# halide/Halide

Measured on AMD Instinct MI355X. Metric: megapixels/sec local_laplacian 8-level fp32 4K, higher is better.
Workload: dtype f32; 1 GPU; apps/local_laplacian J=8 levels=8 alpha=1/7 beta=1, u16 RGB planar 3840x2160; distinct_frames_per_gpu=8, lut_cached=True, streams_per_gpu=4, frame_scheduling=4 frame-queue streams, boundary=C ABI local_laplacian(halide_buffer_t*,int32,float,float,halide_buffer_t*), rccl_ranks=1, parallelism=frames sharded over 1 GPU(s), no data-path collective

## Files before the change

### halide_amd/csrc/local_laplacian.hip

```cpp
#include "hlmi_device_math.h"
#include "hlmi_internal.h"

#include <atomic>
#include <mutex>
#include <optional>
#include <stdlib.h>
#include <string.h>
#include <type_traits>

using namespace hlmi;

namespace {

constexpr int J = 8;
constexpr int MAX_K = 32;
constexpr int STRIP = 126;
constexpr int KCH = 8;
constexpr int D0_THREADS = 256;

struct Level {
    int lox, loy;
    int w, h;
    int ws;
    size_t ps;
// ... 10 lines not shown
#define LL_PROBE_T(var) const unsigned long long var = wall_clock64()
#define LL_PROBE_ADD(slot, val) do { if ((threadIdx.x & 63) == 0) atomicAdd(&g_probe[slot], (unsigned long long)(val)); } while (0)
#else
#define LL_PROBE_T(var)
#define LL_PROBE_ADD(slot, val)
#endif

#ifndef HLMI_LL_RESIDENCY
#define HLMI_LL_RESIDENCY 0
#endif
#if HLMI_LL_RESIDENCY
__device__ int g_res[2][4096];
__device__ unsigned long long g_res_hist[16];
struct ResidencyProbe {
    int kind, slot;
    bool on;
    __device__ explicit ResidencyProbe(int k) : kind(k), slot(0), on(threadIdx.x == 0) {
        if (on) {
            unsigned hw, xcc;
            asm volatile("s_getreg_b32 %0, hwreg(HW_REG_HW_ID)" : "=s"(hw));
            asm volatile("s_getreg_b32 %0, hwreg(HW_REG_XCC_ID)" : "=s"(xcc));
            slot = (int)(((xcc & 0xfu) << 8) | ((hw >> 8) & 0xffu));
            const int own = atomicAdd(&g_res[kind][slot], 1);
            const int other = atomicAdd(&g_res[1 - kind][slot], 0);
            atomicAdd(&g_res_hist[8 * kind + min(other, 3)], 1ull);
            atomicAdd(&g_res_hist[8 * kind + 4 + min(own, 3)], 1ull);
        }
    }
    __device__ ~ResidencyProbe() {
        if (on) atomicSub(&g_res[kind][slot], 1);
    }
};
#define LL_RESIDENCY(kind) ResidencyProbe residency_probe_(kind)
#else
#define LL_RESIDENCY(kind)
#endif

struct Geometry {
    int K, half;
    float Km1, inv_Km1;
    int ix0, ix1, iy0, iy1;
};

__global__ void ll_remap_lut(float *lut, int half, float alpha) {
    int i = blockIdx.x * blockDim.x + threadIdx.x;
    if (i > 2 * half) return;
    float fx = (float)(i - half) * (1.0f / 256.0f);
    lut[i] = (alpha * fx) * dev::halide_exp(((-fx) * fx) * 0.5f);
}

__device__ __forceinline__ int xcd_block() {
    const int nb8 = gridDim.x >> 3, b = blockIdx.x;
    return (b < (nb8 << 3)) ? (b & 7) * nb8 + (b >> 3) : b;
}

__device__ __forceinline__ float down4(float a, float b, float c, float d) {
    return (dev::mad(3.0f, b + c, a) + d) * 0.125f;
}
__device__ __forceinline__ float down4_raw(float a, float b, float c, float d) { return dev::mad(3.0f, b + c, a) + d; }
__device__ __forceinline__ float down4_tail(float a, float b, float c, float d) {
    return (dev::mad(3.0f, b + c, a) + d) * 0.015625f;
}

__device__ __forceinline__ float gray_from(uint16_t r, uint16_t g, uint16_t b) {
    constexpr float s = (float)(1.0 / 65535.0);
    constexpr float C0 = (float)((double)s * (double)0.299f), C1 = (float)((double)s * (double)0.587f),
                    C2 = (float)((double)s * (double)0.114f);
    return dev::mad((float)b, C2, dev::mad2((float)r, C0, (float)g, C1));
// ... 1158 lines not shown
            nc = row(2 * T + 3);
            nd = row(2 * T + 4);
        }
        float dy[4] = {down4_raw(ra.x, rb.x, rc.x, rd.x), down4_raw(ra.y, rb.y, rc.y, rd.y), down4_raw(ra.z, rb.z, rc.z, rd.z),
                       down4_raw(ra.w, rb.w, rc.w, rd.w)};
        float2 o = hpair<ODD>(dy);
        if (store_ok) *reinterpret_cast<float2 *>(dp + (size_t)t * a.dws) = o;
        ra = rc, rb = rd, rc = nc, rd = nd;
    }
}
template<bool ODD>
__global__ __launch_bounds__(256) void ll_down_strip(StripArgs a) {
    const int wave = __builtin_amdgcn_readfirstlane(threadIdx.x >> 6);
    const int unit = xcd_block() * 4 + wave;
    if (unit >= a.nunits) return;
    down_strip_unit<ODD>(a, unit, threadIdx.x & 63);
}

constexpr int S2_RPU = 2;
constexpr int S2_NT = 2 * S2_RPU + 2;
constexpr int S2_NSRC = 2 * S2_NT + 2;
struct Strip2Args {
    const float *src;
    int slox, sloy, sw, sh, sws;
    size_t sps;
    float *g1;
    int so1, loy1, w1, h1, ws1;
    size_t ps1;
    float *g2;
    int so2, loy2, w2, h2, ws2;
    size_t ps2;
    int Pbase, S2, nsx, nsy, nunits;
};
template<bool ODD0, bool ODD1>
__global__ __launch_bounds__(256) void ll_down_strip2(Strip2Args p) {
    const int wave = __builtin_amdgcn_readfirstlane(threadIdx.x >> 6);
    const int unit = xcd_block() * 4 + wave;
    if (unit >= p.nunits) return;
    const int lane = threadIdx.x & 63;
    const int sy = unit % p.nsy, rest = unit / p.nsy, sx = rest % p.nsx, plane = rest / p.nsx;
    const int A = p.loy2 + sy * S2_RPU, B = min(A + S2_RPU - 1, p.loy2 + p.h2 - 1);
    const int P = p.Pbase + 2 * p.S2 * sx + 2 * lane;
    const QuadSel qs = quad_sel((ODD0 ? 2 * P - 1 : 2 * P - 2) - p.slox, p.sw);
    const bool edge_wave = __any(!qs.plain);
    const int T0 = 2 * A - 1;
    const int Ts0 = max(2 * A, p.loy1), Ts1 = min(2 * B + 1, p.loy1 + p.h1 - 1);
    const int off1 = P - p.so1;
    const bool st1_ok = lane < p.S2 && off1 >= 0 && off1 < p.w1;
    const int X2 = ODD1 ? (P + 1) >> 1 : P >> 1;
    const int off2 = X2 - p.so2;
    const bool st2_ok = (ODD1 ? lane < p.S2 : (lane >= 1 && lane <= p.S2)) && off2 >= 0 && off2 < p.w2;
    const float *sp = p.src + (size_t)plane * p.sps + qs.oq;
    float4 r[S2_NSRC];
#pragma unroll
    for (int i = 0; i < S2_NSRC; i++) r[i] = *reinterpret_cast<const float4 *>(sp + (size_t)dev::clampi(2 * T0 - 1 + i - p.sloy, 0, p.sh - 1) * p.sws);
    if (edge_wave) {
#pragma unroll
        for (int i = 0; i < S2_NSRC; i++) {
            const float4 v = r[i];
            r[i] = make_float4(pick4(v.x, v.y, v.z, v.w, qs.sel[0]), pick4(v.x, v.y, v.z, v.w, qs.sel[1]),
                               pick4(v.x, v.y, v.z, v.w, qs.sel[2]), pick4(v.x, v.y, v.z, v.w, qs.sel[3]));
        }
    }
    float *d1 = p.g1 + (size_t)plane * p.ps1 + off1, *d2 = p.g2 + (size_t)plane * p.ps2 + off2;
    float2 s0 = make_float2(0.0f, 0.0f), s1 = s0, pc = s0;
#pragma unroll
    for (int t = 0; t < S2_NT; t++) {
        const int T = T0 + t;
        const float4 a = r[2 * t], b = r[2 * t + 1], c = r[2 * t + 2], d = r[2 * t + 3];
        const float dy[4] = {down4_raw(a.x, b.x, c.x, d.x), down4_raw(a.y, b.y, c.y, d.y), down4_raw(a.z, b.z, c.z, d.z),
                             down4_raw(a.w, b.w, c.w, d.w)};
        const float2 res = hpair<ODD0>(dy);
        if (T >= Ts0 && T <= Ts1 && st1_ok) *reinterpret_cast<float2 *>(d1 + (size_t)(T - p.loy1) * p.ws1) = res;
        if ((t & 1) == 0) {
            pc.x = dev::mad(3.0f, s1.x + res.x, s0.x);
            pc.y = dev::mad(3.0f, s1.y + res.y, s0.y);
            s0 = res;
        } else {
            const float rx = pc.x + res.x, ry = pc.y + res.y;
            float o;
            if (ODD1) {
                const float nx = lane_next(rx), ny = lane_next(ry);
                o = down4_tail(rx, ry, nx, ny);
            } else {
                const float py = lane_prev(ry), nx = lane_next(rx);
                o = down4_tail(py, rx, ry, nx);
            }
            const int Y = (T - 2) >> 1;
            if (T >= 2 * A + 2 && Y <= B && st2_ok) d2[(size_t)(Y - p.loy2) * p.ws2] = o;
            s1 = res;
        }
    }
}


__device__ __forceinline__ float top_value(const float *__restrict__ g, size_t ps, size_t o, int K, float Km1) {
    float level = g[(size_t)K * ps + o] * Km1;
    int li = dev::clampi((int)level, 0, K - 2);
    float lf = level - (float)li;
    return dev::mad2(1.0f - lf, g[(size_t)li * ps + o], lf, g[(size_t)(li + 1) * ps + o]);
}
template<bool SEL = false>
__device__ __forceinline__ float outl_value(const float *__restrict__ g, int ws, size_t ps, int lox, int loy,
                                            const float *__restrict__ gc, int cws, size_t cps, int clox, int cloy,
                                            int X, int Y, int K, float Km1) {
    size_t o = (size_t)(Y - loy) * ws + (X - lox);
    float level = g[(size_t)K * ps + o] * Km1;
    int li = dev::clampi((int)level, 0, K - 2);
    float lf = level - (float)li;
    float l0 = g[(SEL ? 0 : (size_t)li * ps) + o] - up_at(gc + (size_t)li * cps, clox, cloy, cws, X, Y);
    float l1 = g[(SEL ? ps : (size_t)(li + 1) * ps) + o] - up_at(gc + (size_t)(li + 1) * cps, clox, cloy, cws, X, Y);
    return dev::mad2(1.0f - lf, l0, lf, l1);
}

__global__ void ll_top(const float *__restrict__ g, int ws, size_t ps, int lox, int loy, int rx0, int ry0, int rw,
                       int rh, int K, float Km1, float *__restrict__ out) {
    int x = blockIdx.x * blockDim.x + threadIdx.x, y = blockIdx.y;
    if (x >= rw || y >= rh) return;
    size_t o = (size_t)(ry0 + y - loy) * ws + (rx0 + x - lox);
    out[o] = top_value(g, ps, o, K, Km1);
}

// ... 17 lines not shown
    float outL = outl_value<SEL>(a.g, a.ws, a.ps, a.lox, a.loy, a.gc, a.cws, a.cps, a.clox, a.cloy, X, Y, a.K, a.Km1);
    a.out[o] = up_at(a.outc, a.clox, a.cloy, a.cws, X, Y) + outL;
}
template<bool SEL = false>
__global__ __launch_bounds__(256) void ll_up(UpArgs a) {
    up_pixel<SEL>(a, blockIdx.x * blockDim.x + threadIdx.x, blockIdx.y);
}
__global__ __launch_bounds__(256) void ll_up_outl(UpArgs a) {
    const int x = blockIdx.x * blockDim.x + threadIdx.x, y = blockIdx.y;
    if (x >= a.rw || y >= a.rh) return;
    const int X = a.rx0 + x, Y = a.ry0 + y;
    const size_t o = (size_t)(Y - a.loy) * a.ws + (X - a.lox);
    a.out[o] = up_at(a.outc, a.clox, a.cloy, a.cws, X, Y) + a.g[o];
}

struct DevLevel {
    float *g, *out;
    int lox, loy, w, h, ws;
    unsigned ps;
    int rx0, ry0, rw, rh;
};
struct CoarseArgs {
    DevLevel lv[J];
    int K;
    float Km1;
};

constexpr int DM_T = 4;
__host__ __device__ constexpr int dm_win(int depth_below) {
    int w = DM_T;
    for (int i = 0; i < depth_below; i++) w = 2 * w + 2;
    return w;
}
struct Range2 { int x0, x1, y0, y1; };
__device__ __forceinline__ Range2 clamp_to_box(const DevLevel &L, int x0, int x1, int y0, int y1) {
    Range2 r;
    r.x0 = dev::clampi(x0, L.lox, L.lox + L.w - 1), r.x1 = dev::clampi(x1, L.lox, L.lox + L.w - 1);
    r.y0 = dev::clampi(y0, L.loy, L.loy + L.h - 1), r.y1 = dev::clampi(y1, L.loy, L.loy + L.h - 1);
    return r;
}
template<int DEPTH>
__device__ __forceinline__ void down_multi_tile(const CoarseArgs &a, int ntx, int nty, int b) {
    constexpr int W1 = dm_win(DEPTH - 1), W2 = DEPTH >= 2 ? dm_win(DEPTH - 2) : 1, W3 = DEPTH >= 3 ? dm_win(DEPTH - 3) : 1,
                  W4 = DEPTH >= 4 ? dm_win(DEPTH - 4) : 1;
    __shared__ float tile1[W1 * W1], tile2[W2 * W2], tile3[W3 * W3], tile4[W4 * W4];
    float *const tiles[5] = {nullptr, tile1, tile2, tile3, tile4};
    const int ws_[5] = {0, W1, W2, W3, W4};
    const int tx = b % ntx, ty = (b / ntx) % nty, plane = b / (ntx * nty);
    Range2 win[5], own[5];
    {
        const DevLevel &T = a.lv[DEPTH];
        win[DEPTH] = own[DEPTH] = clamp_to_box(T, T.lox + tx * DM_T, T.lox + tx * DM_T + DM_T - 1, T.loy + ty * DM_T,
                                               T.loy + ty * DM_T + DM_T - 1);
#pragma unroll
        for (int d = DEPTH - 1; d >= 1; d--) {
            const DevLevel &L = a.lv[d];
            win[d] = clamp_to_box(L, 2 * win[d + 1].x0 - 1, 2 * win[d + 1].x1 + 2, 2 * win[d + 1].y0 - 1, 2 * win[d + 1].y1 + 2);
            own[d] = clamp_to_box(L, 2 * own[d + 1].x0, 2 * own[d + 1].x1 + 1, 2 * own[d + 1].y0, 2 * own[d + 1].y1 + 1);
        }
    }
#pragma unroll
    for (int d = 1; d <= DEPTH; d++) {
        const DevLevel &L = a.lv[d], &Sx = a.lv[d - 1];
        const Range2 w = win[d], o = own[d];
        const int nx = w.x1 - w.x0 + 1, n = nx * (w.y1 - w.y0 + 1);
        float *const dst = tiles[d];
        const float *const src_g = Sx.g + (size_t)plane * Sx.ps;
        const float *const src_t = tiles[d - 1];
        const Range2 pw = win[d == 1 ? 1 : d - 1];
        const int pnx = ws_[d == 1 ? 1 : d - 1];
        for (int e0 = threadIdx.x; e0 < n; e0 += 512) {
            float r[2][4][4];
            int X[2], Y[2], yy[2];
            bool ok[2];
#pragma unroll
            for (int u = 0; u < 2; u++) {
                const int e = e0 + 256 * u, ec = min(e, n - 1);
                ok[u] = e < n;
                yy[u] = ec / nx, X[u] = w.x0 + (ec - yy[u] * nx), Y[u] = w.y0 + yy[u];
#pragma unroll
                for (int i = 0; i < 4; i++) {
#pragma unroll
                    for (int k = 0; k < 4; k++) {
                        const int qx = dev::clampi(2 * X[u] - 1 + i, Sx.lox, Sx.lox + Sx.w - 1);
                        const int qy = dev::clampi(2 * Y[u] - 1 + k, Sx.loy, Sx.loy + Sx.h - 1);
                        r[u][i][k] = (d == 1) ? src_g[(size_t)(qy - Sx.loy) * Sx.ws + (qx - Sx.lox)]
                                              : src_t[(qy - pw.y0) * pnx + (qx - pw.x0)];
                    }
                }
            }
#pragma unroll
            for (int u = 0; u < 2; u++) {
                float v[4];
#pragma unroll
                for (int i = 0; i < 4; i++) v[i] = down4_raw(r[u][i][0], r[u][i][1], r[u][i][2], r[u][i][3]);
                const float val = down4_tail(v[0], v[1], v[2], v[3]);
                if (ok[u]) {
                    dst[yy[u] * ws_[d] + (X[u] - w.x0)] = val;
                    if (X[u] >= o.x0 && X[u] <= o.x1 && Y[u] >= o.y0 && Y[u] <= o.y1) {
                        L.g[(size_t)plane * L.ps + (size_t)(Y[u] - L.loy) * L.ws + (X[u] - L.lox)] = val;
                    }
                }
            }
        }
        if (d < DEPTH) __syncthreads();
    }
}
template<int DEPTH>
__global__ __launch_bounds__(256) void ll_down_multi(CoarseArgs a, int ntx, int nty) {
    down_multi_tile<DEPTH>(a, ntx, nty, (int)blockIdx.x);
}

constexpr int UM_T = 16;
__host__ __device__ constexpr int um_win(int d) {
    int w = UM_T;
    for (int i = 0; i < d; i++) w = w / 2 + 2;
    return w;
}
__host__ __device__ constexpr int um_off(int d) {
    int o = 0;
    for (int i = 0; i < d; i++) o += um_win(i) * um_win(i);
    return o;
}
static_assert(UM_T * UM_T <= 256 && um_win(1) * um_win(1) <= 256, "ll_up_multi: a level's region of a tile exceeds the workgroup");
template<int TOP>
__device__ __forceinline__ void up_multi_tile(const CoarseArgs &a, int ntx, int b) {
    __shared__ float tl[um_off(TOP + 1)];
    const int tx = b % ntx, ty = b / ntx;
    Range2 reg[TOP + 1];
    {
        const DevLevel &L = a.lv[0];
        reg[0].x0 = L.rx0 + tx * UM_T, reg[0].x1 = min(reg[0].x0 + UM_T - 1, L.rx0 + L.rw - 1);
        reg[0].y0 = L.ry0 + ty * UM_T, reg[0].y1 = min(reg[0].y0 + UM_T - 1, L.ry0 + L.rh - 1);
#pragma unroll
        for (int d = 1; d <= TOP; d++) {
            reg[d].x0 = dev::fdiv2(reg[d - 1].x0 - 1), reg[d].x1 = dev::fdiv2(reg[d - 1].x1 + 1);
            reg[d].y0 = dev::fdiv2(reg[d - 1].y0 - 1), reg[d].y1 = dev::fdiv2(reg[d - 1].y1 + 1);
        }
    }
    int eX[TOP + 1], eY[TOP + 1];
    bool act[TOP + 1];
    size_t eo[TOP + 1];
    float lvl[TOP + 1];
#pragma unroll
    for (int d = 0; d <= TOP; d++) {
        const DevLevel &L = a.lv[d];
        const Range2 r = reg[d];
        const int nx = r.x1 - r.x0 + 1, n = nx * (r.y1 - r.y0 + 1);
        act[d] = (int)threadIdx.x < n;
        const int e = act[d] ? (int)threadIdx.x : 0, yy = e / nx;
        eX[d] = r.x0 + (e - yy * nx), eY[d] = r.y0 + yy;
        eo[d] = (size_t)(eY[d] - L.loy) * L.ws + (eX[d] - L.lox);
        lvl[d] = L.g[(size_t)a.K * L.ps + eo[d]];
    }
    __builtin_amdgcn_sched_barrier(0);
    float lf[TOP + 1], g0[TOP + 1], g1[TOP + 1];
    int lis[TOP + 1];
    UpTaps t0[TOP + 1], t1[TOP + 1];
    auto planes_of = [&](int d) {
        const float level = lvl[d] * a.Km1;
        lis[d] = dev::clampi((int)level, 0, a.K - 2);
        lf[d] = level - (float)lis[d];
    };
#pragma unroll
    for (int d = 0; d <= TOP; d++) {
        const DevLevel &L = a.lv[d];
        planes_of(d);
        const int li = lis[d];
        g0[d] = L.g[(size_t)li * L.ps + eo[d]], g1[d] = L.g[(size_t)(li + 1) * L.ps + eo[d]];
        if (d < TOP) {
            const DevLevel &C = a.lv[d + 1];
            t0[d] = up_taps(C.g + (size_t)li * C.ps, C.lox, C.loy, C.ws, eX[d], eY[d]);
            t1[d] = up_taps(C.g + (size_t)(li + 1) * C.ps, C.lox, C.loy, C.ws, eX[d], eY[d]);
        }
    }
    __builtin_amdgcn_sched_barrier(0);
#pragma unroll
    for (int d = 0; d <= TOP; d++) {
        float v;
        if (d == TOP) {
            v = dev::mad2(1.0f - lf[d], g0[d], lf[d], g1[d]);
        } else {
            const float l0 = g0[d] - up_from(t0[d], eX[d], eY[d]);
            const float l1 = g1[d] - up_from(t1[d], eX[d], eY[d]);
            v = dev::mad2(1.0f - lf[d], l0, lf[d], l1);
        }
        if (act[d]) (tl + um_off(d))[(eY[d] - reg[d].y0) * um_win(d) + (eX[d] - reg[d].x0)] = v;
    }
    __syncthreads();
#pragma unroll
    for (int d = TOP - 1; d >= 0; d--) {
        const Range2 r = reg[d], c = reg[d + 1];
        const float *const ct = tl + um_off(d + 1);
        float *const tile = tl + um_off(d);
        const int cw = um_win(d + 1), tw = um_win(d);
        const int nx = r.x1 - r.x0 + 1, n = nx * (r.y1 - r.y0 + 1);
        for (int e = threadIdx.x; e < n; e += 256) {
            const int yy = e / nx, X = r.x0 + (e - yy * nx), Y = r.y0 + yy;
            const int xa = dev::fdiv2(X + 1) - c.x0, xb = dev::fdiv2(X - 1) - c.x0;
            const int ya = dev::fdiv2(Y + 1) - c.y0, yb = dev::fdiv2(Y - 1) - c.y0;
            const float wx = (float)(dev::fmod2(X) * 2 + 1) * 0.25f, wy = (float)(dev::fmod2(Y) * 2 + 1) * 0.25f;
            const float ua = dev::lerpf(ct[ya * cw + xa], ct[ya * cw + xb], wx);
            const float ub = dev::lerpf(ct[yb * cw + xa], ct[yb * cw + xb], wx);
            const float v = dev::lerpf(ua, ub, wy) + tile[yy * tw + (X - r.x0)];
            if (d == 0) {
                const DevLevel &L = a.lv[0];
                L.out[(size_t)(Y - L.loy) * L.ws + (X - L.lox)] = v;
            } else {
                tile[yy * tw + (X - r.x0)] = v;
            }
        }
        if (d > 0) __syncthreads();
    }
}
template<int TOP>
__global__ __launch_bounds__(256) void ll_up_multi(CoarseArgs a, int ntx) {
    up_multi_tile<TOP>(a, ntx, (int)blockIdx.x);
}



struct Up0Args {
    const uint16_t *in;
    long in_sy;
    long gco[3];
    long cco[3];
    const float *lut_g, *g1, *out1;
    int lox1, loy1, ws1;
    size_t ps1;
    uint16_t *out;
    long out_sy, out_sc;
    int ox0, oy0, ow, oh, nc, RU;
    int same_ch;
    float beta;
    const float *g2, *out2;
    int lox2, loy2, ws2;
    size_t ps2;
    int rx1_1;
    int rx0_1, ry0_1, ry1_1;
};

template<bool VEC, bool LUT_LDS>
__global__ __launch_bounds__(256) void ll_up0(Up0Args p, Geometry gm) {
    extern __shared__ float slut[];
    if (LUT_LDS) {
        for (int i = threadIdx.x; i <= 2 * gm.half; i += 256) slut[i] = p.lut_g[i];
        __syncthreads();
    }
    const float *lut = LUT_LDS ? slut : p.lut_g;
    const int wave = threadIdx.x >> 6, lane = threadIdx.x & 63;
// ... 479 lines not shown
            float q[3];
            div3_by(n, gr, q);
#pragma unroll
            for (int c = 0; c < 3; c++) res[c][i] = (uint16_t)__builtin_amdgcn_fmed3f(q[c], 0.0f, 65535.0f);
        }
        if (y < y1) {
            uint16_t *orow = p.out + (long)y * p.out_sy;
#pragma unroll
            for (int c = 0; c < 3; c++) st_frame2<NT>(reinterpret_cast<char *>(orow + (long)c * p.out_sc) + fresh(outb), res[c][0], res[c][1]);
        }
    };
    Frame f[U0H_PF];
#pragma unroll
    for (int i = 0; i < U0H_PF; i++) load_frame(y0 + i, f[i]);
    for (int y = y0; y < y1; y += U0H_PF) {
#pragma unroll
        for (int i = 0; i < U0H_PF; i++) {
            const Frame cur = f[i];
            load_frame(y + U0H_PF + i, f[i]);
            finish(y + i, cur);
        }
    }
}

const ArgTable ll_table("local_laplacian", {
    in_buf("input", T_U16, 3, {0, 1536, 0, 2560, 0, 3}),
    scalar_i32("levels").estimate(8),
    scalar_f32("alpha").estimate(1),
    scalar_f32("beta").estimate(1),
    out_buf("output", T_U16, 3, {0, 1536, 0, 2560, 0, 3}),
});

struct LlSwitches {
    std::optional<int> fuse_from, upchain_from, ru, units0, no_vec, emit, nt, fuse_up2, d01_exch, d01_pad_lds, no_lut_cache, emit1;
};
LlSwitches ll_switches() {
    const auto get = env_int;
    LlSwitches s;
    s.fuse_from = get("HLMI_LL_FUSE_FROM"), s.upchain_from = get("HLMI_LL_UPCHAIN_FROM");
    s.ru = get("HLMI_LL_RU"), s.units0 = get("HLMI_LL_UNITS0"), s.no_vec = get("HLMI_LL_NO_VEC");
    s.emit = get("HLMI_LL_EMIT"), s.nt = get("HLMI_LL_NT"), s.fuse_up2 = get("HLMI_LL_FUSE_UP2");
    s.d01_exch = get("HLMI_LL_D01_EXCH"), s.d01_pad_lds = get("HLMI_LL_D01_PAD_LDS"), s.no_lut_cache = get("HLMI_LL_NO_LUT_CACHE");
    s.emit1 = get("HLMI_LL_EMIT1");
    return s;
}

int dev_clamp_ru(int ru) { return ru < 1 ? 1 : (ru > 300 ? 300 : ru); }

struct PairGeom {
    int S2;
    int Pbase;
    int nsx;
};
struct LlPlan {
    Geometry gm;
    Level lv[J];
    size_t off_g[J], off_out[J], off_l0, ws_floats;
    Up0Args u0;
    int nlut;
    int S, SU;
    int up_low;
    bool lut_cache;
    bool lut_lds;
    bool vec_frame;
    bool vec_in;
    bool b1;
    bool fast, fuse1, fuse2, emit, nt;
    bool emit1;
    bool d01;
    bool strip2;
    struct { PairGeom pg; bool exch; int nsy, nunits; size_t lds; } d0;
    struct { PairGeom pg; int nsy, nunits; } s2;
    int units_strip;
    size_t up0_lds;
};

struct LlBuffers {
    float *lut, *outl0;
    float *g[J], *outg[J];
};

PairGeom pair_geom(const Level &d, const Level &e, int fewer = 0) {
    PairGeom g;
    g.S2 = ((d.odd || e.odd) ? 62 : 61) - fewer;
    const int lim = e.odd ? 2 * e.lox - 1 : 2 * e.lox - 2;
    g.Pbase = min(d.lox, lim);
    const int hi1 = d.lox + d.w - 1, hi2 = e.lox + e.w - 1;
    const int x2_first = e.odd ? (g.Pbase + 1) / 2 + 0 : g.Pbase / 2 + 1;
    g.nsx = max((hi2 - x2_first + g.S2) / g.S2, (hi1 - g.Pbase + 2 * g.S2) / (2 * g.S2));
    return g;
}

void ll_plan(LlPlan &pl, const halide_buffer_t *input, const halide_buffer_t *output, int levels, float beta, const LlSwitches &sw,
             int stream_cus, int device_cus) {
    Up0Args &p = pl.u0;
    const int ow = p.ow = output->dim[0].extent, oh = p.oh = output->dim[1].extent, nc = p.nc = output->dim[2].extent;
    Geometry &gm = pl.gm;
    gm.K = levels;
    gm.half = (levels - 1) * 256;
    gm.Km1 = (float)(levels - 1);
    gm.inv_Km1 = 1.0f / gm.Km1;
    gm.ix0 = input->dim[0].min, gm.ix1 = gm.ix0 + input->dim[0].extent - 1;
    gm.iy0 = input->dim[1].min, gm.iy1 = gm.iy0 + input->dim[1].extent - 1;
// ... 112 lines not shown
        int nwy = 0;
        auto ceil_div = [](int x, int y) { return (x + y - 1) / y; };
        if (exch) {
            const int nwy_max = max(1, target2 / (WPB * pg.nsx));
            const int n = max(2, (ceil_div(e.h, nwy_max) + 1 + 3) / 4);
            nwy = ceil_div(e.h, 4 * n - 1);
            exch = e.h / nwy >= 4;
        }
        pl.d0.exch = exch;
        if (exch) {
            pl.d0.nsy = nwy;
            pl.d0.nunits = pg.nsx * nwy * WPB;
        } else {
            pl.d0.nsy = max(1, min(max(target2 / pg.nsx, (e.h + 31) / 32), e.h));
            pl.d0.nunits = pg.nsx * pl.d0.nsy;
        }
        size_t sh2 = sizeof(float) * ((nlut + 1) & ~1) + sizeof(float2) * D01_STATE * (WPB + (exch ? WPB - 1 : 0));
        if (pl.emit1) sh2 += d01_em1_lds_bytes();
        const int pad = sw.d01_pad_lds.value_or(emit && partitioned ? -1 : 0);
        constexpr size_t kHalfCuLds = 160 * 1024 / 2;
        if (pad < 0) sh2 = max(sh2, kHalfCuLds + 2048);
        else sh2 += (size_t)pad;
        pl.d0.lds = sh2;
    }
    if (pl.strip2) {
        pl.s2.pg = pair_geom(lv[3], lv[4]);
        pl.s2.nsy = (lv[4].h + S2_RPU - 1) / S2_RPU;
        pl.s2.nunits = (levels + 1) * pl.s2.pg.nsx * pl.s2.nsy;
    }
    pl.units_strip = 16 * device_cus;
    pl.up0_lds = emit   ? sizeof(float) * ((size_t)U0_TS * (RU + 2) + (size_t)U0H_T2 * (RU / 2 + 4))
                 : fast ? lut_sh + (fuse1 ? ((lut_lds && (nlut & 1)) ? 4 : 0) + sizeof(float) * U0_TS * (RU + 2) : 0)
                        : lut_sh;
}

struct LlLastCall {
    LlPlan pl;
    LlBuffers b;
    hipStream_t stream;
    bool out1_pending;
    bool out2_pending;
};
thread_local LlLastCall t_dbg = {};

StripArgs strip_args(const LlPlan &pl, const LlBuffers &b, int j) {
    const Level &sl = pl.lv[j], &d = pl.lv[j + 1];
    const int cols = d.nsx * (pl.gm.K + 1);
    StripArgs a;
    a.src = b.g[j], a.slox = sl.lox, a.sloy = sl.loy, a.sw = sl.w, a.sh = sl.h, a.sws = sl.ws, a.sps = sl.ps;
    a.dst = b.g[j + 1], a.Xs = d.lox, a.dloy = d.loy, a.dw = d.w, a.dh = d.h, a.dws = d.ws, a.dps = d.ps;
    a.nsx = d.nsx;
    a.nsy = max(1, min(max(pl.units_strip / cols, (d.h + 31) / 32), max(1, d.h / 2)));
    a.nunits = cols * a.nsy;
    return a;
}
CoarseArgs coarse_args(const LlPlan &pl, const LlBuffers &b, int from) {
    CoarseArgs ca;
    for (int dl = 0; from + dl < J; dl++) {
        const Level &L = pl.lv[from + dl];
        DevLevel &D = ca.lv[dl];
        D.g = b.g[from + dl], D.out = b.outg[from + dl], D.lox = L.lox, D.loy = L.loy, D.w = L.w, D.h = L.h, D.ws = L.ws, D.ps = (unsigned)L.ps;
        D.rx0 = L.rx0, D.ry0 = L.ry0, D.rw = L.rx1 - L.rx0 + 1, D.rh = L.ry1 - L.ry0 + 1;
    }
    ca.K = pl.gm.K, ca.Km1 = pl.gm.Km1;
    return ca;
}
// ... 60 lines not shown
    dim3 grid((a.nunits + WPB - 1) / WPB);
    if (pl.emit) {
        timing_note_bytes(6.0 * iw * (gm.iy1 - gm.iy0 + 1) + 4.0 * iw * f.oh + 4.0 * (pl.emit1 ? 1.0 : 3.0) * d.w * d.h +
                          4.0 * (levels + 1) * e.w * e.h);
        D01EArgs ae;
        ae.d = a, ae.outl0 = b.outl0, ae.oy0 = f.oy0, ae.oh = f.oh;
        ae.nsx_magic = a.nsx == 1 ? 0u : (unsigned)((1ull << 32) / (unsigned)a.nsx + 1ull);
        ae.last2 = e.loy + e.h - 1;
        return with_flags([&](auto O0, auto O1, auto B, auto EX, auto NT, auto E1) -> int {
            HLMI_LAUNCH(uc, "ll_down01", st, (ll_down01e<O0.value, O1.value, B.value, EX.value, NT.value, E1.value>), grid, block, pl.d0.lds, ae,
                        gm, lev);
            return 0;
        }, d.odd, e.odd, pl.b1, pl.d0.exch, pl.nt, pl.emit1);
    }
    timing_note_bytes(d0_bytes + 4.0 * (levels + 1) * e.w * e.h);
    return with_flags([&](auto O0, auto O1, auto B, auto EX) -> int {
        HLMI_LAUNCH(uc, "ll_down01", st, (ll_down01f<O0.value, O1.value, B.value, EX.value>), grid, block, pl.d0.lds, a, gm, lev);
        return 0;
    }, d.odd, e.odd, pl.b1, pl.d0.exch);
}

int ll_stage_down_rest(void *uc, const LlPlan &pl, const LlBuffers &b, hipStream_t st) {
    const Level *lv = pl.lv;
    const int levels = pl.gm.K, S = pl.S;
    if (pl.strip2) {
        const Level &sl = lv[2], &d = lv[3], &e = lv[4];
        Strip2Args a;
        a.src = b.g[2], a.slox = sl.lox, a.sloy = sl.loy, a.sw = sl.w, a.sh = sl.h, a.sws = sl.ws, a.sps = sl.ps;
        a.g1 = b.g[3], a.so1 = d.lox, a.loy1 = d.loy, a.w1 = d.w, a.h1 = d.h, a.ws1 = d.ws, a.ps1 = d.ps;
        a.g2 = b.g[4], a.so2 = e.lox, a.loy2 = e.loy, a.w2 = e.w, a.h2 = e.h, a.ws2 = e.ws, a.ps2 = e.ps;
        a.S2 = pl.s2.pg.S2, a.Pbase = pl.s2.pg.Pbase, a.nsx = pl.s2.pg.nsx, a.nsy = pl.s2.nsy, a.nunits = pl.s2.nunits;
        timing_note_bytes(4.0 * (levels + 1) * ((double)sl.w * sl.h + (double)d.w * d.h + (double)e.w * e.h));
        dim3 grid((a.nunits + 3) / 4), block(256);
        if (int r = with_flags([&](auto O0, auto O1) -> int {
                HLMI_LAUNCH(uc, "ll_down_strip2:2", st, (ll_down_strip2<O0.value, O1.value>), grid, block, 0, a);
                return 0;
            }, d.odd, e.odd)) return r;
    }
    for (int j = 1; j + 1 < J; j++) {
        if (pl.strip2 && (j == 2 || j == 3)) continue;
        if (j == S) {
            const CoarseArgs ca = coarse_args(pl, b, S);
            long total = 0;
            for (int dl = 1; S + dl < J; dl++) total += (long)(levels + 1) * lv[S + dl].w * lv[S + dl].h;
            const int ntx = (lv[J - 1].w + DM_T - 1) / DM_T, nty = (lv[J - 1].h + DM_T - 1) / DM_T;
            dim3 grid((unsigned)(ntx * nty * (levels + 1))), block(256);
            char nm[32];
            snprintf(nm, sizeof nm, "ll_down_multi:%d", S);
            timing_note_bytes(4.0 * ((double)(levels + 1) * lv[S].w * lv[S].h + (double)total));
            if (J - 1 - S == 4) HLMI_LAUNCH(uc, nm, st, (ll_down_multi<4>), grid, block, 0, ca, ntx, nty);
            else if (J - 1 - S == 3) HLMI_LAUNCH(uc, nm, st, (ll_down_multi<3>), grid, block, 0, ca, ntx, nty);
            else if (J - 1 - S == 2) HLMI_LAUNCH(uc, nm, st, (ll_down_multi<2>), grid, block, 0, ca, ntx, nty);
            else HLMI_LAUNCH(uc, nm, st, (ll_down_multi<1>), grid, block, 0, ca, ntx, nty);
            break;
        }
        if (j == 1 && pl.d01) continue;
        const StripArgs sa = strip_args(pl, b, j);
        dim3 grid((sa.nunits + 3) / 4), block(256);
        char nm[32];
        snprintf(nm, sizeof nm, "ll_down_strip:%d", j);
        timing_note_bytes(4.0 * (levels + 1) * ((double)lv[j].w * lv[j].h + (double)lv[j + 1].w * lv[j + 1].h));
        if (int r = with_flags([&](auto O) -> int {
                HLMI_LAUNCH(uc, nm, st, (ll_down_strip<O.value>), grid, block, 0, sa);
                return 0;
            }, lv[j + 1].odd)) return r;
    }
    return 0;
}

int ll_stage_up_coarse(void *uc, const LlPlan &pl, const LlBuffers &b, hipStream_t st) {
    const Level *lv = pl.lv;
    const int levels = pl.gm.K, SU = pl.SU;
    if (SU < J) {
        const CoarseArgs cu = coarse_args(pl, b, SU);
        const int ntx = (cu.lv[0].rw + UM_T - 1) / UM_T, nty = (cu.lv[0].rh + UM_T - 1) / UM_T;
        dim3 grid((unsigned)(ntx * nty)), block(256);
        char nm[32];
        snprintf(nm, sizeof nm, "ll_up_multi:%d", SU);
        {
            const double px = (double)cu.lv[0].rw * cu.lv[0].rh;
            timing_note_bytes(4.0 * 4.0 * px * (SU + 1 < J ? 4.0 / 3.0 : 1.0));
        }
        switch (J - 1 - SU) {
#define LL_UM(T) case T: HLMI_LAUNCH(uc, nm, st, (ll_up_multi<T>), grid, block, 0, cu, ntx); break;
            LL_UM(1) LL_UM(2) LL_UM(3) LL_UM(4) LL_UM(5) LL_UM(6)
#undef LL_UM
        }
    } else {
        const Level &t = lv[J - 1];
        int rw = t.rx1 - t.rx0 + 1, rh = t.ry1 - t.ry0 + 1;
        HLMI_LAUNCH(uc, "ll_top", st, ll_top, dim3((rw + 63) / 64, rh), dim3(64), 0, b.g[J - 1], t.ws, t.ps, t.lox, t.loy, t.rx0,
                    t.ry0, rw, rh, levels, pl.gm.Km1, b.outg[J - 1]);
    }
    for (int j = min(SU, J - 1) - 1; j >= pl.up_low; j--) {
        const UpArgs ua = up_args(pl, b, j);
        char nm[32];
        snprintf(nm, sizeof nm, "ll_up:%d", j);
        timing_note_bytes(4.0 * (4.0 * ua.rw * ua.rh + 3.0 * (lv[j + 1].rx1 - lv[j + 1].rx0 + 1) * (lv[j + 1].ry1 - lv[j + 1].ry0 + 1)));
        HLMI_LAUNCH(uc, nm, st, ll_up<false>, dim3((ua.rw + 255) / 256, ua.rh), dim3(256), 0, ua);
    }
    return 0;
}

int ll_stage_up0(void *uc, const LlPlan &pl, const LlBuffers &b, hipStream_t st) {
    const Geometry &gm = pl.gm;
    const Level *lv = pl.lv;
    const Level &c = lv[1];
    Up0Args p = pl.u0;
    const int ow = p.ow, oh = p.oh, nc = p.nc;
    p.lut_g = b.lut, p.g1 = b.g[1], p.out1 = b.outg[1];
    p.lox1 = c.lox, p.loy1 = c.loy, p.ws1 = c.ws, p.ps1 = c.ps;
    p.g2 = b.g[2], p.out2 = b.outg[2], p.lox2 = lv[2].lox, p.loy2 = lv[2].loy, p.ws2 = lv[2].ws, p.ps2 = lv[2].ps;
    p.rx1_1 = c.rx1, p.rx0_1 = c.rx0, p.ry0_1 = c.ry0, p.ry1_1 = c.ry1;
    dim3 grid((ow + 255) / 256, (oh + 2 * p.RU - 1) / (2 * p.RU)), block(256);
    const double n1 = (double)(c.rx1 - c.rx0 + 1) * (c.ry1 - c.ry0 + 1), n2 = (double)(lv[2].rx1 - lv[2].rx0 + 1) * (lv[2].ry1 - lv[2].ry0 + 1);
    if (pl.emit) {
        timing_note_bytes(2.0 * (3 + nc) * ow * oh + 4.0 * ow * oh + 4.0 * (pl.emit1 ? 1.0 : 3.0) * n1 + 4.0 * 3.0 * n2);
// ... 80 lines not shown
    table.done(st);
    mark_output_written(output);
    return 0;
}

HLMI_ENTRY_AUTO(local_laplacian, ll_table.md)

extern "C" int hlmi_debug_ll_probe(unsigned long long *out32) {
#if HLMI_LL_PROBE
    if (hipDeviceSynchronize() != hipSuccess) return -1;
    if (hipMemcpyFromSymbol(out32, HIP_SYMBOL(g_probe), sizeof(unsigned long long) * 32) != hipSuccess) return -1;
    unsigned long long zero[32] = {};
    if (hipMemcpyToSymbol(HIP_SYMBOL(g_probe), zero, sizeof zero) != hipSuccess) return -1;
    return 1;
#else
    (void)out32;
    return 0;
#endif
}

extern "C" int hlmi_debug_ll_residency(unsigned long long *out16) {
#if HLMI_LL_RESIDENCY
    if (hipDeviceSynchronize() != hipSuccess) return -1;
    if (hipMemcpyFromSymbol(out16, HIP_SYMBOL(g_res_hist), sizeof(unsigned long long) * 16) != hipSuccess) return -1;
    unsigned long long zero[16] = {};
    if (hipMemcpyToSymbol(HIP_SYMBOL(g_res_hist), zero, sizeof zero) != hipSuccess) return -1;
    return 1;
#else
    (void)out16;
    return 0;
#endif
}

extern "C" int hlmi_debug_dpp_probe(void) {
    int *flag = nullptr, h = 0;
    if (hipMalloc(&flag, sizeof(int)) != hipSuccess) return -1;
    if (hipMemset(flag, 0, sizeof(int)) != hipSuccess) return -1;
    hipLaunchKernelGGL(ll_dpp_probe, dim3(1), dim3(64), 0, 0, flag);
    if (hipMemcpy(&h, flag, sizeof(int), hipMemcpyDeviceToHost) != hipSuccess) return -1;
    (void)hipFree(flag);
    return h;
}

extern "C" int hlmi_debug_div3_check(const float *n, const float *d, int count) {
    float *dn = nullptr, *dd = nullptr;
    int *bad = nullptr, h = -1;
    if (hipMalloc(&dn, sizeof(float) * count) != hipSuccess || hipMalloc(&dd, sizeof(float) * count) != hipSuccess ||
        hipMalloc(&bad, sizeof(int)) != hipSuccess) {
        return -1;
    }
    if (hipMemcpy(dn, n, sizeof(float) * count, hipMemcpyHostToDevice) != hipSuccess ||
        hipMemcpy(dd, d, sizeof(float) * count, hipMemcpyHostToDevice) != hipSuccess ||
        hipMemset(bad, 0, sizeof(int)) != hipSuccess) {
        return -1;
    }
    hipLaunchKernelGGL(ll_div3_check, dim3((count + 255) / 256), dim3(256), 0, 0, dn, dd, count, bad);
    if (hipMemcpy(&h, bad, sizeof(int), hipMemcpyDeviceToHost) != hipSuccess) h = -1;
    (void)hipFree(dn), (void)hipFree(dd), (void)hipFree(bad);
    return h;
}

extern "C" int hlmi_debug_local_laplacian_outg(int level, float *dst, int cap_floats, int *rw_out, int *rh_out) {
    LlLastCall &c = t_dbg;
    if (level < 1 || level >= J || !c.b.outg[level]) return -1;
    const Level &L = c.pl.lv[level];
    int rw = L.rx1 - L.rx0 + 1, rh = L.ry1 - L.ry0 + 1;
// ... 35 lines not shown
```

Measured before the change: 119,500 Mpx/s.

## Add register-fit variants of coarse down/up chain kernels with 32-bit offsets

```diff
diff --git a/halide_amd/csrc/local_laplacian.hip b/halide_amd/csrc/local_laplacian.hip
--- a/halide_amd/csrc/local_laplacian.hip
+++ b/halide_amd/csrc/local_laplacian.hip
@@ -66,8 +66,41 @@
     }
 };
 #define LL_RESIDENCY(kind) ResidencyProbe residency_probe_(kind)
+__device__ unsigned long long g_chain_hist[3][2][4], g_chain_span[3][3], g_chain_first[3][16], g_chain_key[16];
+__device__ unsigned g_chain_count[3][16];
+__device__ __forceinline__ void chain_probe(int chain, const void *key, unsigned nwg) {
+    if (threadIdx.x != 0) return;
+    const unsigned long long t = wall_clock64();
+    unsigned hw, xcc;
+    asm volatile("s_getreg_b32 %0, hwreg(HW_REG_HW_ID)" : "=s"(hw));
+    asm volatile("s_getreg_b32 %0, hwreg(HW_REG_XCC_ID)" : "=s"(xcc));
+    const int slot = (int)(((xcc & 0xfu) << 8) | ((hw >> 8) & 0xffu));
+    for (int kind = 0; kind < 2; kind++) atomicAdd(&g_chain_hist[chain][kind][min(atomicAdd(&g_res[kind][slot], 0), 3)], 1ull);
+    int q = 0;
+    for (; q < 15; q++) {
+        const unsigned long long was = atomicCAS(&g_chain_key[q], 0ull, (unsigned long long)key);
+        if (was == 0ull || was == (unsigned long long)key) break;
+    }
+    const unsigned rank = atomicAdd(&g_chain_count[chain][q], 1u) % nwg;
+    if (rank == 0) atomicExch(&g_chain_first[chain][q], t);
+    if (rank == nwg - 1) {
+        const unsigned long long first = atomicAdd(&g_chain_first[chain][q], 0ull), span = t > first ? t - first : 0ull;
+        atomicAdd(&g_chain_span[chain][0], 1ull), atomicAdd(&g_chain_span[chain][1], span), atomicMax(&g_chain_span[chain][2], span);
+    }
+}
+#define LL_CHAIN_RESIDENCY(chain, key) chain_probe(chain, key, gridDim.x)
 #else
 #define LL_RESIDENCY(kind)
+#define LL_CHAIN_RESIDENCY(chain, key)
+#endif
+
+#ifndef HLMI_LL_CHAIN_PRIO
+#define HLMI_LL_CHAIN_PRIO 0
+#endif
+#if HLMI_LL_CHAIN_PRIO
+#define LL_CHAIN_PRIO() __builtin_amdgcn_s_setprio(HLMI_LL_CHAIN_PRIO)
+#else
+#define LL_CHAIN_PRIO()
 #endif
 
 struct Geometry {
@@ -1292,8 +1325,11 @@
     size_t ps2;
     int Pbase, S2, nsx, nsy, nunits;
 };
-template<bool ODD0, bool ODD1>
+constexpr int S2_FIT_NSRC = 8, S2_FIT_NSRC_ODD = 7;
+template<bool ODD0, bool ODD1, bool FIT = false>
 __global__ __launch_bounds__(256) void ll_down_strip2(Strip2Args p) {
+    LL_CHAIN_PRIO();
+    LL_CHAIN_RESIDENCY(0, p.g1);
     const int wave = __builtin_amdgcn_readfirstlane(threadIdx.x >> 6);
     const int unit = xcd_block() * 4 + wave;
     if (unit >= p.nunits) return;
@@ -1311,27 +1347,57 @@
     const int off2 = X2 - p.so2;
     const bool st2_ok = (ODD1 ? lane < p.S2 : (lane >= 1 && lane <= p.S2)) && off2 >= 0 && off2 < p.w2;
     const float *sp = p.src + (size_t)plane * p.sps + qs.oq;
-    float4 r[S2_NSRC];
-#pragma unroll
-    for (int i = 0; i < S2_NSRC; i++) r[i] = *reinterpret_cast<const float4 *>(sp + (size_t)dev::clampi(2 * T0 - 1 + i - p.sloy, 0, p.sh - 1) * p.sws);
-    if (edge_wave) {
-#pragma unroll
-        for (int i = 0; i < S2_NSRC; i++) {
-            const float4 v = r[i];
-            r[i] = make_float4(pick4(v.x, v.y, v.z, v.w, qs.sel[0]), pick4(v.x, v.y, v.z, v.w, qs.sel[1]),
-                               pick4(v.x, v.y, v.z, v.w, qs.sel[2]), pick4(v.x, v.y, v.z, v.w, qs.sel[3]));
+    constexpr int NR = !FIT ? S2_NSRC : ODD0 ? S2_FIT_NSRC_ODD : S2_FIT_NSRC;
+    float4 r[NR];
+    const float *const su = p.src + (size_t)plane * p.sps;
+    const uint32_t lane_off = 4u * (uint32_t)qs.oq;
+    auto request = [&](int i) {
+        const size_t row = (size_t)dev::clampi(2 * T0 - 1 + i - p.sloy, 0, p.sh - 1) * p.sws;
+        return *reinterpret_cast<const float4 *>(reinterpret_cast<const char *>(su + row) + lane_off);
+    };
+    auto select = [&](float4 &v) {
+        v = make_float4(pick4(v.x, v.y, v.z, v.w, qs.sel[0]), pick4(v.x, v.y, v.z, v.w, qs.sel[1]),
+                        pick4(v.x, v.y, v.z, v.w, qs.sel[2]), pick4(v.x, v.y, v.z, v.w, qs.sel[3]));
+    };
+    if constexpr (FIT) {
+#pragma unroll
+        for (int i = 0; i < NR; i++) r[i] = request(i);
+    } else {
+#pragma unroll
+        for (int i = 0; i < S2_NSRC; i++) r[i] = *reinterpret_cast<const float4 *>(sp + (size_t)dev::clampi(2 * T0 - 1 + i - p.sloy, 0, p.sh - 1) * p.sws);
+        if (edge_wave) {
+#pragma unroll
+            for (int i = 0; i < S2_NSRC; i++) {
+                const float4 v = r[i];
+                r[i] = make_float4(pick4(v.x, v.y, v.z, v.w, qs.sel[0]), pick4(v.x, v.y, v.z, v.w, qs.sel[1]),
+                                   pick4(v.x, v.y, v.z, v.w, qs.sel[2]), pick4(v.x, v.y, v.z, v.w, qs.sel[3]));
+            }
         }
     }
     float *d1 = p.g1 + (size_t)plane * p.ps1 + off1, *d2 = p.g2 + (size_t)plane * p.ps2 + off2;
+    float *const u1 = p.g1 + (size_t)plane * p.ps1, *const u2 = p.g2 + (size_t)plane * p.ps2;
     float2 s0 = make_float2(0.0f, 0.0f), s1 = s0, pc = s0;
 #pragma unroll
     for (int t = 0; t < S2_NT; t++) {
         const int T = T0 + t;
-        const float4 a = r[2 * t], b = r[2 * t + 1], c = r[2 * t + 2], d = r[2 * t + 3];
+        if (FIT && edge_wave) {
+#pragma unroll
+            for (int i = (t == 0 ? 0 : 2 * t + 2); i < 2 * t + 4; i++) select(r[i % NR]);
+        }
+        const float4 a = r[(2 * t) % NR], b = r[(2 * t + 1) % NR], c = r[(2 * t + 2) % NR], d = r[(2 * t + 3) % NR];
         const float dy[4] = {down4_raw(a.x, b.x, c.x, d.x), down4_raw(a.y, b.y, c.y, d.y), down4_raw(a.z, b.z, c.z, d.z),
                              down4_raw(a.w, b.w, c.w, d.w)};
+        if (FIT && 2 * t + NR < S2_NSRC) {
+            __builtin_amdgcn_sched_barrier(0);
+            r[(2 * t) % NR] = request(2 * t + NR);
+            if (2 * t + 1 + NR < S2_NSRC) r[(2 * t + 1) % NR] = request(2 * t + 1 + NR);
+            __builtin_amdgcn_sched_barrier(0);
+        }
         const float2 res = hpair<ODD0>(dy);
-        if (T >= Ts0 && T <= Ts1 && st1_ok) *reinterpret_cast<float2 *>(d1 + (size_t)(T - p.loy1) * p.ws1) = res;
+        if (T >= Ts0 && T <= Ts1 && st1_ok) {
+            if constexpr (FIT) *reinterpret_cast<float2 *>(reinterpret_cast<char *>(u1 + (size_t)(T - p.loy1) * p.ws1) + 4u * (uint32_t)off1) = res;
+            else *reinterpret_cast<float2 *>(d1 + (size_t)(T - p.loy1) * p.ws1) = res;
+        }
         if ((t & 1) == 0) {
             pc.x = dev::mad(3.0f, s1.x + res.x, s0.x);
             pc.y = dev::mad(3.0f, s1.y + res.y, s0.y);
@@ -1347,7 +1413,10 @@
                 o = down4_tail(py, rx, ry, nx);
             }
             const int Y = (T - 2) >> 1;
-            if (T >= 2 * A + 2 && Y <= B && st2_ok) d2[(size_t)(Y - p.loy2) * p.ws2] = o;
+            if (T >= 2 * A + 2 && Y <= B && st2_ok) {
+                if constexpr (FIT) *reinterpret_cast<float *>(reinterpret_cast<char *>(u2 + (size_t)(Y - p.loy2) * p.ws2) + 4u * (uint32_t)off2) = o;
+                else d2[(size_t)(Y - p.loy2) * p.ws2] = o;
+            }
             s1 = res;
         }
     }
@@ -1431,6 +1500,11 @@
     for (int i = 0; i < depth_below; i++) w = 2 * w + 2;
     return w;
 }
+__host__ __device__ constexpr size_t dm_lds_bytes(int depth) {
+    size_t n = 0;
+    for (int below = 1; below < depth; below++) n += (size_t)dm_win(below) * dm_win(below);
+    return sizeof(float) * n;
+}
 struct Range2 { int x0, x1, y0, y1; };
 __device__ __forceinline__ Range2 clamp_to_box(const DevLevel &L, int x0, int x1, int y0, int y1) {
     Range2 r;
@@ -1438,7 +1512,7 @@
     r.y0 = dev::clampi(y0, L.loy, L.loy + L.h - 1), r.y1 = dev::clampi(y1, L.loy, L.loy + L.h - 1);
     return r;
 }
-template<int DEPTH>
+template<int DEPTH, bool FIT = false>
 __device__ __forceinline__ void down_multi_tile(const CoarseArgs &a, int ntx, int nty, int b) {
     constexpr int W1 = dm_win(DEPTH - 1), W2 = DEPTH >= 2 ? dm_win(DEPTH - 2) : 1, W3 = DEPTH >= 3 ? dm_win(DEPTH - 3) : 1,
                   W4 = DEPTH >= 4 ? dm_win(DEPTH - 4) : 1;
@@ -1483,8 +1557,13 @@
                     for (int k = 0; k < 4; k++) {
                         const int qx = dev::clampi(2 * X[u] - 1 + i, Sx.lox, Sx.lox + Sx.w - 1);
                         const int qy = dev::clampi(2 * Y[u] - 1 + k, Sx.loy, Sx.loy + Sx.h - 1);
-                        r[u][i][k] = (d == 1) ? src_g[(size_t)(qy - Sx.loy) * Sx.ws + (qx - Sx.lox)]
-                                              : src_t[(qy - pw.y0) * pnx + (qx - pw.x0)];
+                        if (FIT && d == 1) {
+                            r[u][i][k] = *reinterpret_cast<const float *>(reinterpret_cast<const char *>(src_g) +
+                                                                          4u * (uint32_t)((qy - Sx.loy) * Sx.ws + (qx - Sx.lox)));
+                        } else {
+                            r[u][i][k] = (d == 1) ? src_g[(size_t)(qy - Sx.loy) * Sx.ws + (qx - Sx.lox)]
+                                                  : src_t[(qy - pw.y0) * pnx + (qx - pw.x0)];
+                        }
                     }
                 }
             }
@@ -1507,7 +1586,15 @@
 }
 template<int DEPTH>
 __global__ __launch_bounds__(256) void ll_down_multi(CoarseArgs a, int ntx, int nty) {
+    LL_CHAIN_PRIO();
+    LL_CHAIN_RESIDENCY(1, a.lv[1].g);
     down_multi_tile<DEPTH>(a, ntx, nty, (int)blockIdx.x);
+}
+template<int DEPTH>
+__global__ __launch_bounds__(256) void ll_down_multi_fit(CoarseArgs a, int ntx, int nty) {
+    LL_CHAIN_PRIO();
+    LL_CHAIN_RESIDENCY(1, a.lv[1].g);
+    down_multi_tile<DEPTH, true>(a, ntx, nty, (int)blockIdx.x);
 }
 
 constexpr int UM_T = 16;
@@ -1521,8 +1608,9 @@
     for (int i = 0; i < d; i++) o += um_win(i) * um_win(i);
     return o;
 }
+__host__ __device__ constexpr size_t um_lds_bytes(int top) { return sizeof(float) * um_off(top + 1); }
 static_assert(UM_T * UM_T <= 256 && um_win(1) * um_win(1) <= 256, "ll_up_multi: a level's region of a tile exceeds the workgroup");
-template<int TOP>
+template<int TOP, bool FIT = false>
 __device__ __forceinline__ void up_multi_tile(const CoarseArgs &a, int ntx, int b) {
     __shared__ float tl[um_off(TOP + 1)];
     const int tx = b % ntx, ty = b / ntx;
@@ -1537,54 +1625,88 @@
             reg[d].y0 = dev::fdiv2(reg[d - 1].y0 - 1), reg[d].y1 = dev::fdiv2(reg[d - 1].y1 + 1);
         }
     }
-    int eX[TOP + 1], eY[TOP + 1];
-    bool act[TOP + 1];
-    size_t eo[TOP + 1];
-    float lvl[TOP + 1];
-#pragma unroll
-    for (int d = 0; d <= TOP; d++) {
-        const DevLevel &L = a.lv[d];
-        const Range2 r = reg[d];
-        const int nx = r.x1 - r.x0 + 1, n = nx * (r.y1 - r.y0 + 1);
-        act[d] = (int)threadIdx.x < n;
-        const int e = act[d] ? (int)threadIdx.x : 0, yy = e / nx;
-        eX[d] = r.x0 + (e - yy * nx), eY[d] = r.y0 + yy;
-        eo[d] = (size_t)(eY[d] - L.loy) * L.ws + (eX[d] - L.lox);
-        lvl[d] = L.g[(size_t)a.K * L.ps + eo[d]];
-    }
-    __builtin_amdgcn_sched_barrier(0);
-    float lf[TOP + 1], g0[TOP + 1], g1[TOP + 1];
-    int lis[TOP + 1];
-    UpTaps t0[TOP + 1], t1[TOP + 1];
-    auto planes_of = [&](int d) {
-        const float level = lvl[d] * a.Km1;
-        lis[d] = dev::clampi((int)level, 0, a.K - 2);
-        lf[d] = level - (float)lis[d];
-    };
-#pragma unroll
-    for (int d = 0; d <= TOP; d++) {
-        const DevLevel &L = a.lv[d];
-        planes_of(d);
-        const int li = lis[d];
-        g0[d] = L.g[(size_t)li * L.ps + eo[d]], g1[d] = L.g[(size_t)(li + 1) * L.ps + eo[d]];
-        if (d < TOP) {
-            const DevLevel &C = a.lv[d + 1];
-            t0[d] = up_taps(C.g + (size_t)li * C.ps, C.lox, C.loy, C.ws, eX[d], eY[d]);
-            t1[d] = up_taps(C.g + (size_t)(li + 1) * C.ps, C.lox, C.loy, C.ws, eX[d], eY[d]);
-        }
-    }
-    __builtin_amdgcn_sched_barrier(0);
-#pragma unroll
-    for (int d = 0; d <= TOP; d++) {
-        float v;
-        if (d == TOP) {
-            v = dev::mad2(1.0f - lf[d], g0[d], lf[d], g1[d]);
-        } else {
-            const float l0 = g0[d] - up_from(t0[d], eX[d], eY[d]);
-            const float l1 = g1[d] - up_from(t1[d], eX[d], eY[d]);
-            v = dev::mad2(1.0f - lf[d], l0, lf[d], l1);
-        }
-        if (act[d]) (tl + um_off(d))[(eY[d] - reg[d].y0) * um_win(d) + (eX[d] - reg[d].x0)] = v;
+    auto at = [](const float *g, size_t o) -> float {
+        if constexpr (FIT) return *reinterpret_cast<const float *>(reinterpret_cast<const char *>(g) + 4u * (uint32_t)o);
+        else return g[o];
+    };
+    auto levels_lo_hi = [&](auto lo_c, auto hi_c) {
+        constexpr int LO = decltype(lo_c)::value, HI = decltype(hi_c)::value, N = HI - LO + 1;
+        int eX[N], eY[N];
+        bool act[N];
+        size_t eo[N];
+        float lvl[N];
+#pragma unroll
+        for (int d = LO; d <= HI; d++) {
+            const int i = d - LO;
+            const DevLevel &L = a.lv[d];
+            const Range2 r = reg[d];
+            const int nx = r.x1 - r.x0 + 1, n = nx * (r.y1 - r.y0 + 1);
+            act[i] = (int)threadIdx.x < n;
+            const int e = act[i] ? (int)threadIdx.x : 0, yy = e / nx;
+            eX[i] = r.x0 + (e - yy * nx), eY[i] = r.y0 + yy;
+            eo[i] = (size_t)(eY[i] - L.loy) * L.ws + (eX[i] - L.lox);
+            lvl[i] = at(L.g, (size_t)a.K * L.ps + eo[i]);
+        }
+        __builtin_amdgcn_sched_barrier(0);
+        float lf[N], g0[N], g1[N];
+        int lis[N];
+        UpTaps t0[N], t1[N];
+        auto planes_of = [&](int i) {
+            const float level = lvl[i] * a.Km1;
+            lis[i] = dev::clampi((int)level, 0, a.K - 2);
+            lf[i] = level - (float)lis[i];
+        };
+#pragma unroll
+        for (int d = LO; d <= HI; d++) {
+            const int i = d - LO;
+            const DevLevel &L = a.lv[d];
+            planes_of(i);
+            const int li = lis[i];
+            g0[i] = at(L.g, (size_t)li * L.ps + eo[i]), g1[i] = at(L.g, (size_t)(li + 1) * L.ps + eo[i]);
+            if (d < TOP) {
+                const DevLevel &C = a.lv[d + 1];
+                if constexpr (FIT) {
+                    const int xa = dev::fdiv2(eX[i] + 1) - C.lox, xb = dev::fdiv2(eX[i] - 1) - C.lox;
+                    const int ya = dev::fdiv2(eY[i] + 1) - C.loy, yb = dev::fdiv2(eY[i] - 1) - C.loy;
+                    const size_t p0 = (size_t)li * C.ps, p1 = (size_t)(li + 1) * C.ps;
+                    t0[i].aa = at(C.g, p0 + ya * C.ws + xa), t0[i].ab = at(C.g, p0 + ya * C.ws + xb);
+                    t0[i].ba = at(C.g, p0 + yb * C.ws + xa), t0[i].bb = at(C.g, p0 + yb * C.ws + xb);
+                    t1[i].aa = at(C.g, p1 + ya * C.ws + xa), t1[i].ab = at(C.g, p1 + ya * C.ws + xb);
+                    t1[i].ba = at(C.g, p1 + yb * C.ws + xa), t1[i].bb = at(C.g, p1 + yb * C.ws + xb);
+                } else {
+                    t0[i] = up_taps(C.g + (size_t)li * C.ps, C.lox, C.loy, C.ws, eX[i], eY[i]);
+                    t1[i] = up_taps(C.g + (size_t)(li + 1) * C.ps, C.lox, C.loy, C.ws, eX[i], eY[i]);
+                }
+            }
+        }
+        __builtin_amdgcn_sched_barrier(0);
+#pragma unroll
+        for (int d = LO; d <= HI; d++) {
+            const int i = d - LO;
+            float v;
+            if (d == TOP) {
+                v = dev::mad2(1.0f - lf[i], g0[i], lf[i], g1[i]);
+            } else {
+                const float l0 = g0[i] - up_from(t0[i], eX[i], eY[i]);
+                const float l1 = g1[i] - up_from(t1[i], eX[i], eY[i]);
+                v = dev::mad2(1.0f - lf[i], l0, lf[i], l1);
+            }
+            if (act[i]) (tl + um_off(d))[(eY[i] - reg[d].y0) * um_win(d) + (eX[i] - reg[d].x0)] = v;
+        }
+    };
+    if constexpr (FIT && TOP >= 5) {
+        levels_lo_hi(std::integral_constant<int, 0>{}, std::integral_constant<int, 1>{});
+        __builtin_amdgcn_sched_barrier(0);
+        levels_lo_hi(std::integral_constant<int, 2>{}, std::integral_constant<int, 3>{});
+        __builtin_amdgcn_sched_barrier(0);
+        levels_lo_hi(std::integral_constant<int, 4>{}, std::integral_constant<int, TOP>{});
+    } else if constexpr (FIT) {
+        constexpr int GS = (TOP + 1) / 2;
+        levels_lo_hi(std::integral_constant<int, 0>{}, std::integral_constant<int, GS - 1>{});
+        __builtin_amdgcn_sched_barrier(0);
+        levels_lo_hi(std::integral_constant<int, GS>{}, std::integral_constant<int, TOP>{});
+    } else {
+        levels_lo_hi(std::integral_constant<int, 0>{}, std::integral_constant<int, TOP>{});
     }
     __syncthreads();
 #pragma unroll
@@ -1614,7 +1736,15 @@
 }
 template<int TOP>
 __global__ __launch_bounds__(256) void ll_up_multi(CoarseArgs a, int ntx) {
+    LL_CHAIN_PRIO();
+    LL_CHAIN_RESIDENCY(2, a.lv[0].out);
     up_multi_tile<TOP>(a, ntx, (int)blockIdx.x);
+}
+template<int TOP>
+__global__ __launch_bounds__(256) void ll_up_multi_fit(CoarseArgs a, int ntx) {
+    LL_CHAIN_PRIO();
+    LL_CHAIN_RESIDENCY(2, a.lv[0].out);
+    up_multi_tile<TOP, true>(a, ntx, (int)blockIdx.x);
 }
 
 
@@ -2160,7 +2290,7 @@
 });
 
 struct LlSwitches {
-    std::optional<int> fuse_from, upchain_from, ru, units0, no_vec, emit, nt, fuse_up2, d01_exch, d01_pad_lds, no_lut_cache, emit1;
+    std::optional<int> fuse_from, upchain_from, ru, units0, no_vec, emit, nt, fuse_up2, d01_exch, d01_pad_lds, no_lut_cache, emit1, chain_fit;
 };
 LlSwitches ll_switches() {
     const auto get = env_int;
@@ -2169,7 +2299,7 @@
     s.ru = get("HLMI_LL_RU"), s.units0 = get("HLMI_LL_UNITS0"), s.no_vec = get("HLMI_LL_NO_VEC");
     s.emit = get("HLMI_LL_EMIT"), s.nt = get("HLMI_LL_NT"), s.fuse_up2 = get("HLMI_LL_FUSE_UP2");
     s.d01_exch = get("HLMI_LL_D01_EXCH"), s.d01_pad_lds = get("HLMI_LL_D01_PAD_LDS"), s.no_lut_cache = get("HLMI_LL_NO_LUT_CACHE");
-    s.emit1 = get("HLMI_LL_EMIT1");
+    s.emit1 = get("HLMI_LL_EMIT1"), s.chain_fit = get("HLMI_LL_CHAIN_FIT");
     return s;
 }
 
@@ -2197,6 +2327,7 @@
     bool emit1;
     bool d01;
     bool strip2;
+    bool chain_fit;
     struct { PairGeom pg; bool exch; int nsy, nunits; size_t lds; } d0;
     struct { PairGeom pg; int nsy, nunits; } s2;
     int units_strip;
@@ -2375,6 +2506,12 @@
     pl.up0_lds = emit   ? sizeof(float) * ((size_t)U0_TS * (RU + 2) + (size_t)U0H_T2 * (RU / 2 + 4))
                  : fast ? lut_sh + (fuse1 ? ((lut_lds && (nlut & 1)) ? 4 : 0) + sizeof(float) * U0_TS * (RU + 2) : 0)
                         : lut_sh;
+    {
+        const int cf = (double)(levels + 1) * (4.0 * (double)lv[1].ps) < 4.0e9 ? sw.chain_fit.value_or(-1) : 0;
+        const size_t taken = lds_alloc(pl.d0.lds) + 3 * lds_alloc(pl.up0_lds);
+        const size_t need = max(S < J - 1 ? lds_alloc(dm_lds_bytes(J - 1 - S)) : (size_t)0, SU < J - 1 ? lds_alloc(um_lds_bytes(J - 1 - SU)) : (size_t)0);
+        pl.chain_fit = cf > 0 || (cf < 0 && pl.emit1 && partitioned && taken + need <= kCuLds);
+    }
 }
 
 struct LlLastCall {
@@ -2501,10 +2638,10 @@
         a.S2 = pl.s2.pg.S2, a.Pbase = pl.s2.pg.Pbase, a.nsx = pl.s2.pg.nsx, a.nsy = pl.s2.nsy, a.nunits = pl.s2.nunits;
         timing_note_bytes(4.0 * (levels + 1) * ((double)sl.w * sl.h + (double)d.w * d.h + (double)e.w * e.h));
         dim3 grid((a.nunits + 3) / 4), block(256);
-        if (int r = with_flags([&](auto O0, auto O1) -> int {
-                HLMI_LAUNCH(uc, "ll_down_strip2:2", st, (ll_down_strip2<O0.value, O1.value>), grid, block, 0, a);
+        if (int r = with_flags([&](auto O0, auto O1, auto F) -> int {
+                HLMI_LAUNCH(uc, "ll_down_strip2:2", st, (ll_down_strip2<O0.value, O1.value, F.value>), grid, block, 0, a);
                 return 0;
-            }, d.odd, e.odd)) return r;
+            }, d.odd, e.odd, pl.chain_fit)) return r;
     }
     for (int j = 1; j + 1 < J; j++) {
         if (pl.strip2 && (j == 2 || j == 3)) continue;
@@ -2517,10 +2654,12 @@
             char nm[32];
             snprintf(nm, sizeof nm, "ll_down_multi:%d", S);
             timing_note_bytes(4.0 * ((double)(levels + 1) * lv[S].w * lv[S].h + (double)total));
-            if (J - 1 - S == 4) HLMI_LAUNCH(uc, nm, st, (ll_down_multi<4>), grid, block, 0, ca, ntx, nty);
-            else if (J - 1 - S == 3) HLMI_LAUNCH(uc, nm, st, (ll_down_multi<3>), grid, block, 0, ca, ntx, nty);
-            else if (J - 1 - S == 2) HLMI_LAUNCH(uc, nm, st, (ll_down_multi<2>), grid, block, 0, ca, ntx, nty);
-            else HLMI_LAUNCH(uc, nm, st, (ll_down_multi<1>), grid, block, 0, ca, ntx, nty);
+            switch ((J - 1 - S) * 2 + (pl.chain_fit ? 1 : 0)) {
+#define LL_DM(D) case 2 * D: HLMI_LAUNCH(uc, nm, st, (ll_down_multi<D>), grid, block, 0, ca, ntx, nty); break; \
+                 case 2 * D + 1: HLMI_LAUNCH(uc, nm, st, (ll_down_multi_fit<D>), grid, block, 0, ca, ntx, nty); break;
+                LL_DM(1) LL_DM(2) LL_DM(3) LL_DM(4)
+#undef LL_DM
+            }
             break;
         }
         if (j == 1 && pl.d01) continue;
@@ -2550,8 +2689,9 @@
             const double px = (double)cu.lv[0].rw * cu.lv[0].rh;
             timing_note_bytes(4.0 * 4.0 * px * (SU + 1 < J ? 4.0 / 3.0 : 1.0));
         }
-        switch (J - 1 - SU) {
-#define LL_UM(T) case T: HLMI_LAUNCH(uc, nm, st, (ll_up_multi<T>), grid, block, 0, cu, ntx); break;
+        switch ((J - 1 - SU) * 2 + (pl.chain_fit ? 1 : 0)) {
+#define LL_UM(T) case 2 * T: HLMI_LAUNCH(uc, nm, st, (ll_up_multi<T>), grid, block, 0, cu, ntx); break; \
+                 case 2 * T + 1: HLMI_LAUNCH(uc, nm, st, (ll_up_multi_fit<T>), grid, block, 0, cu, ntx); break;
             LL_UM(1) LL_UM(2) LL_UM(3) LL_UM(4) LL_UM(5) LL_UM(6)
 #undef LL_UM
         }
@@ -2698,6 +2838,21 @@
 #endif
 }
 
+extern "C" int hlmi_debug_ll_chain_residency(unsigned long long *out33) {
+#if HLMI_LL_RESIDENCY
+    if (hipDeviceSynchronize() != hipSuccess) return -1;
+    if (hipMemcpyFromSymbol(out33, HIP_SYMBOL(g_chain_hist), sizeof(unsigned long long) * 24) != hipSuccess) return -1;
+    if (hipMemcpyFromSymbol(out33 + 24, HIP_SYMBOL(g_chain_span), sizeof(unsigned long long) * 9) != hipSuccess) return -1;
+    unsigned long long zero[24] = {};
+    if (hipMemcpyToSymbol(HIP_SYMBOL(g_chain_hist), zero, sizeof(unsigned long long) * 24) != hipSuccess) return -1;
+    if (hipMemcpyToSymbol(HIP_SYMBOL(g_chain_span), zero, sizeof(unsigned long long) * 9) != hipSuccess) return -1;
+    return 1;
+#else
+    (void)out33;
+    return 0;
+#endif
+}
+
 extern "C" int hlmi_debug_dpp_probe(void) {
     int *flag = nullptr, h = 0;
     if (hipMalloc(&flag, sizeof(int)) != hipSuccess) return -1;
```

Result: faster. 121,900 Mpx/s (median of 6 runs) (+2.0%).
